# aptx4869lm/4DCapture-FPV

Measured on AMD Instinct MI355X. Metric: frames/sec global-opt (fixed iters), 1024f clip/500k-pt scene; Chamfer GB/s, higher is better.
Workload: dtype f32; 1 GPU; BASELINE config 3: 1024-frame clip, 500000-pt scene, 500 contact verts, 500 Adam iterations (phase split 0.8), full loss; frames sharded over 1 GPU(s); frames=1024, scene_points=500000, contact_verts=500, iters=500, body_verts=10475, lbs_weights_per_vertex=4

## Files before the change

4dcapture-fpv_amd/capi.py:

```python
from __future__ import annotations

import ctypes
import os
from ctypes import POINTER, c_char_p, c_double, c_float, c_int32, c_int64, c_void_p

import numpy as np

_HERE = os.path.dirname(os.path.abspath(__file__))
LIB_PATH = os.environ.get("FDCAP_LIB") or os.path.join(_HERE, "libfdcap_hip.so")

NUM_LOSSES = 8
XDIM = 78
PDIM = 75


class FdcapError(RuntimeError):
    pass


class ModelDesc(ctypes.Structure):
    _fields_ = [("num_verts", c_int32), ("v_template", POINTER(c_float)), ("shapedirs", POINTER(c_float)),
                ("num_shape", c_int32), ("posedirs", POINTER(c_float)), ("J_regressor", POINTER(c_float)),
                ("parents", POINTER(c_int32)), ("lbs_weights", POINTER(c_float)),
                ("hands_componentsl", POINTER(c_float)), ("hands_componentsr", POINTER(c_float)),
# ... 74 lines not shown
    "fdcap_opt_backward_dct": (c_int32, [c_void_p, c_float, c_float, c_float, c_int32, c_void_p]),
    "fdcap_opt_set_dct_coef": (c_int32, [c_void_p, c_void_p, c_void_p]),
    "fdcap_opt_get_dct": (c_int32, [c_void_p, c_void_p, c_void_p]),
    "fdcap_opt_get_dct_state": (c_int32, [c_void_p, c_void_p, c_void_p, c_void_p]),
    "fdcap_opt_set_dct_state": (c_int32, [c_void_p, c_void_p, c_void_p, c_void_p]),
    "fdcap_opt_dct_windows": (c_int32, [c_void_p, POINTER(c_int32), POINTER(c_int32)]),
    "fdcap_frame_smoother": (c_int32, [c_void_p, c_void_p, c_int32, c_int32, c_float, c_float, c_float, c_float,
                                        c_void_p, c_int32, c_int32, c_void_p, c_void_p]),
    "fdcap_opt_set_keypoints": (c_int32, [c_void_p, c_void_p, c_void_p]),
    "fdcap_opt_backward_fit2d": (c_int32, [c_void_p, POINTER(Fit2dStage), c_int32, c_void_p]),
    "fdcap_opt_reset_adam": (c_int32, [c_void_p, c_void_p]),
    "fdcap_lbfgs_create": (c_int32, [c_int32, POINTER(LbfgsConfig), POINTER(c_void_p)]),
    "fdcap_lbfgs_destroy": (None, [c_void_p]),
    "fdcap_lbfgs_reset": (c_int32, [c_void_p, c_void_p]),
    "fdcap_lbfgs_advance": (c_int32, [c_void_p, c_void_p, c_int32, c_void_p, c_void_p, c_int32, c_void_p, c_void_p]),
    "fdcap_lbfgs_get_stats": (c_int32, [c_void_p, c_void_p, c_void_p, c_void_p, c_void_p]),
    "fdcap_lbfgs_finalize": (c_int32, [c_void_p, c_void_p, c_int32, c_void_p, c_void_p]),
    "fdcap_opt_fit2d_lbfgs": (c_int32, [c_void_p, POINTER(Fit2dStage), POINTER(LbfgsConfig), c_int32, POINTER(c_int32), c_void_p]),
    "fdcap_opt_fit2d_lbfgs_stats": (c_int32, [c_void_p, c_void_p, c_void_p, c_void_p, c_void_p]),
    "fdcap_opt_step_rows_and_pack": (c_int32, [c_void_p, c_int32, c_int32, c_void_p, c_void_p]),
    "fdcap_opt_unpack_and_step_scale": (c_int32, [c_void_p, c_int32, c_int32, c_void_p, c_int32, c_int32, c_void_p]),
    "fdcap_opt_forward_ahead": (c_int32, [c_void_p, c_int32, c_int32, c_int32, c_void_p]),
    "fdcap_exchange_len": (c_int32, []),
    "fdcap_opt_get_results": (c_int32, [c_void_p, c_void_p, c_void_p, c_void_p, c_void_p]),
    "fdcap_opt_destroy": (None, [c_void_p]),
    "fdcap_opt_forward_world": (c_int32, [c_void_p, c_void_p, c_void_p, c_void_p]),
    "fdcap_opt_get_contact": (c_int32, [c_void_p, c_void_p, c_void_p, c_void_p]),
    "fdcap_opt_get_grads": (c_int32, [c_void_p, c_void_p, c_void_p, c_void_p]),
    "fdcap_panel_gemm": (c_int32, [c_void_p, c_int32, c_int32, c_int32, c_void_p, c_int64, c_int64, c_int32, c_void_p, c_int32,
                                   c_void_p]),
    "fdcap_time_blend_gemm": (c_int32, [c_void_p, c_int32, c_int32, POINTER(c_float), c_void_p]),
    "fdcap_opt_nn_timing": (c_int32, [c_void_p, c_int32]),
    "fdcap_opt_nn_timing_read": (c_int32, [c_void_p, POINTER(c_float), POINTER(c_int32)]),
    "fdcap_opt_launch_timing": (c_int32, [c_void_p, c_int32]),
    "fdcap_opt_launch_timing_read": (c_int32, [c_void_p, c_void_p, c_void_p]),
    "fdcap_opt_time_chamfer": (c_int32, [c_void_p, c_int32, c_int32, POINTER(c_float), c_void_p]),
}

_lib = None


def load_library(path: str | None = None) -> ctypes.CDLL:
    global _lib
    if _lib is not None and path is None:
        return _lib
    p = path or LIB_PATH
    if not os.path.exists(p):
        raise FdcapError(f"{p} is missing: build it with `python -c 'import __graft_entry__ as g; g.build()'` "
                         "(hipcc --offload-arch=gfx950).  There is no CPU fallback.")
    lib = ctypes.CDLL(p)
    for name, (res, args) in SYMBOLS.items():
        fn = getattr(lib, name)
        fn.restype = res
        fn.argtypes = args
    info = lib.fdcap_build_info().decode()
    if "packed_fp32=off" not in info and os.environ.get("FDCAP_ALLOW_PK_F32") != "1":
        raise FdcapError(f"{p} was built with packed fp32 instructions ({info}): results are not reliable next to another kernel's "
                         "MFMAs on the same CU (NOTES.md section 6).  Rebuild with __graft_entry__.build(), or set "
                         "FDCAP_ALLOW_PK_F32=1 for an instrumentation variant.")
    if path is None:
        _lib = lib
    return lib


def count_packed_fp32(path: str | None = None) -> int:
    import re
# ... 107 lines not shown
```

4dcapture-fpv_amd/csrc/fdc_api_opt.h:

```cpp
#pragma once

extern "C" {

void fdcap_opt_destroy(fdcap_ctx* c) {
    if (!c || !c->opt) return;
    OptState* o = c->opt;
    DevBuf<float>* fb[] = {&o->X0, &o->mask, &o->mX, &o->vX, &o->mCAM, &o->vCAM, &o->mS, &o->vS,
                           &o->H1, &o->H2, &o->O, &o->dO, &o->Opart, &o->dZpart, &o->Rm, &o->PF, &o->Jrest, &o->G, &o->A, &o->M,
                           &o->Jw, &o->Voff, &o->Vw, &o->dist, &o->pd, &o->dVoff, &o->dA, &o->dtransl_v, &o->dMv,
                           &o->dsv, &o->dPF, &o->dJw, &o->dX, &o->dCAM, &o->dscale_row, &o->loss_rows, &o->VoffF, &o->VwF, &o->dVF};
    for (auto* b : fb) b->release();
    o->dctD.release(); o->dctCoef.release(); o->dctM.release(); o->dctV.release(); o->adam_tab.release();
    o->idx.release(); o->pi.release(); o->seedpt.release(); o->kp2d.release(); o->floss.release();
    if (o->lbfgs) { fdcap_lbfgs_destroy(o->lbfgs); o->lbfgs = nullptr; }
    o->nnc_ids.release(); o->nnc_hdr.release(); o->nnc_anchor.release();
    for (hipEvent_t e : o->nn_ev) (void)hipEventDestroy(e);
    o->nn_ev.clear();
    for (hipEvent_t e : o->lt.ev) (void)hipEventDestroy(e);
    o->lt.ev.clear(); o->lt.what.clear(); o->lt.on = false; o->lt.used = 0;
    delete o;
    c->opt = nullptr;
}

int fdcap_opt_create(fdcap_ctx* c, const fdcap_opt_config* cfg, float* rows_x, float* rows_cam, float* scale_d,
// ... 30 lines not shown
    AL(o->X0, (size_t)R * XDIM) AL(o->mask, R)
    AL(o->mX, (size_t)R * XDIM) AL(o->vX, (size_t)R * XDIM) AL(o->mCAM, (size_t)R * 16) AL(o->vCAM, (size_t)R * 16)
    AL(o->mS, 1) AL(o->vS, 1)
    AL(o->H1, (size_t)R * 512) AL(o->H2, (size_t)R * 512) AL(o->O, (size_t)R * O_LD) AL(o->dO, (size_t)R * ODIM)
    AL(o->Opart, (size_t)4 * R * ODIM) AL(o->dZpart, (size_t)4 * R * VP_Z)
    AL(o->Rm, (size_t)R * RM_LD) AL(o->PF, (size_t)R * NPFX) AL(o->Jrest, (size_t)R * JR_LD) AL(o->G, (size_t)R * NJ * 12)
    AL(o->A, (size_t)R * NJ * 12) AL(o->M, (size_t)R * 12) AL(o->Jw, (size_t)R * NJW * 3)
    AL(o->dA, (size_t)R * NJ * 12) AL(o->dtransl_v, (size_t)R * 3) AL(o->dMv, (size_t)R * 12)
    AL(o->dsv, R) AL(o->dPF, (size_t)2 * R * NPFX)
    AL(o->dJw, (size_t)R * NJW * 3) AL(o->dX, (size_t)R * XDIM)
    AL(o->dCAM, (size_t)R * 16) AL(o->dscale_row, R) AL(o->loss_rows, (size_t)R * LROW)
    if (o->contact_on) {
        AL(o->Voff, nq * 3) AL(o->Vw, nq * 3) AL(o->dist, nq) AL(o->idx, nq) AL(o->dVoff, nq * 3) AL(o->seedpt, nq)
        AL(o->pd, (size_t)std::max(o->nsplit, o->nsplit_bf) * nq) AL(o->pi, (size_t)std::max(o->nsplit, o->nsplit_bf) * nq)
    }
#undef AL
    tr.mark("buffers");
    if (!err && o->contact_on) {
        hipError_t e_ = hipMemset(o->idx.p, 0xFF, nq * sizeof(int));
        if (e_ != hipSuccess) err = (int)e_;
    }
    if (!err && o->contact_on) {
        if (const char* e = getenv("FDCAP_SKIN_VEC")) o->skin_vec = e[0] != '0';
        if (const char* e = getenv("FDCAP_FUSE_SKIN")) o->fuse_skin = e[0] != '0';
        if (const char* e = getenv("FDCAP_NN_CACHE_SLACK")) o->nnc_slack = (float)atof(e);
        int every = 32;
        if (const char* e = getenv("FDCAP_NN_ORDER")) every = atoi(e);
        o->nn_order = NNOrder{};
        if (o->nnc_slack > 0.f) {
            const size_t ng = ((size_t)nq_all + 31) / 32, ng4 = ng * 4;
            hipError_t e_ = o->nnc_ids.ensure(ng4 * NN_CACHE_CAP);
            if (e_ == hipSuccess) e_ = o->nnc_hdr.ensure(ng4 + 3 * ng);
            if (e_ == hipSuccess) e_ = o->nnc_anchor.ensure((size_t)4 * nq_all);
            if (e_ == hipSuccess) e_ = hipMemset(o->nnc_hdr.p, 0xFF, ng4 * sizeof(int));
            if (e_ == hipSuccess) e_ = hipMemset(o->nnc_hdr.p + ng4, 0, 3 * ng * sizeof(int));
            if (e_ == hipSuccess) e_ = hipMemset(o->nnc_anchor.p, 0, (size_t)4 * nq_all * sizeof(float4));
            if (e_ != hipSuccess) err = (int)e_;
            if (every > 0) { o->nn_order.on = true; o->nn_order.every = every; }
        }
    }
    if (!err) {
        float s = cfg->scale_init;
        hipError_t e_ = hipMemcpy(o->scale.p, &s, sizeof(float), hipMemcpyHostToDevice);
        if (e_ != hipSuccess) err = (int)e_;
    }
    tr.mark("search state");
    if (err) { fdcap_opt_destroy(c); return err; }
    return FDCAP_OK;
}

int fdcap_opt_set_inputs(fdcap_ctx* c, const float* data78, const float* init78, const float* mask, const float* cam,
                         void* stream) {
    if (!c || !c->opt || !data78 || !init78 || !mask || !cam) return FDCAP_E_ARG;
    { int es_ = opt_sync(c, (hipStream_t)stream); if (es_) return es_; }
    OptState* o = c->opt;
    hipStream_t st = (hipStream_t)stream;
    const size_t n = o->cfg.n_local;
    o->log_pending = false; o->log_dst = nullptr;
    HIP_TRY(hipMemcpyAsync(o->X0.p + 2 * XDIM, data78, n * XDIM * sizeof(float), hipMemcpyDeviceToDevice, st));
    HIP_TRY(hipMemcpyAsync(o->X.p + 2 * XDIM, init78, n * XDIM * sizeof(float), hipMemcpyDeviceToDevice, st));
    HIP_TRY(hipMemcpyAsync(o->mask.p + 2, mask, n * sizeof(float), hipMemcpyDeviceToDevice, st));
    HIP_TRY(hipMemcpyAsync(o->CAM.p + 2 * 16, cam, n * 16 * sizeof(float), hipMemcpyDeviceToDevice, st));
    return FDCAP_OK;
}

static int opt_contact_forward(fdcap_ctx* c, hipStream_t st, bool blend_done = false) {
    OptState* o = c->opt;
    const int nl = o->cfg.n_local, nc = c->nc;
    const size_t off = (size_t)2 * nc * 3;
    const SkinModel smf = c->contact.model();
    const bool fused = !blend_done && o->fuse_skin && gemm_split3_enabled() && c->contact.pn_fwdS.f && smf.vpack && smf.K <= 4 && nl >= clip_forms_min_rows() &&
// ... 190 lines not shown
    if (!c || !c->opt) return FDCAP_E_STATE;
    const fdcap_opt_config& cf = c->opt->cfg;
    const bool phase2 = ii >= P;
    LossWeights lw;
    lw.rec = 1.f;
    lw.smooth = phase2 ? cf.phase2_smooth : cf.phase1_smooth;
    lw.contact = phase2 ? 0.f : cf.phase1_contact;
    lw.world = phase2 ? cf.phase2_world : 0.f;
    lw.dct = 0.f;
    lw.world_on = phase2;
    return opt_backward_impl(c, lw, log_terms, (hipStream_t)stream);
}

int fdcap_opt_backward_and_step(fdcap_ctx* c, int32_t ii, int32_t P, int32_t log_terms, void* stream) {
    if (!c || !c->opt) return FDCAP_E_STATE;
    OptState* o = c->opt;
    const fdcap_opt_config& cf = o->cfg;
    const bool fuse = cf.frame0 == 0 && cf.n_local == cf.n_total && o->dctW == 0;
    if (!fuse) {
        const int e = fdcap_opt_backward(c, ii, P, log_terms, stream);
        return e ? e : fdcap_opt_step(c, ii, P, stream);
    }
    const bool phase2 = ii >= P;
    LossWeights lw;
    lw.rec = 1.f;
    lw.smooth = phase2 ? cf.phase2_smooth : cf.phase1_smooth;
    lw.contact = phase2 ? 0.f : cf.phase1_contact;
    lw.world = phase2 ? cf.phase2_world : 0.f;
    lw.dct = 0.f;
    lw.world_on = phase2;
    return opt_backward_impl(c, lw, log_terms, (hipStream_t)stream, ii, P);
}

}
```

4dcapture-fpv_amd/csrc/fdc_chamfer.h:

```cpp
#pragma once
#include <hip/hip_runtime.h>
#include <stdlib.h>

#include <atomic>

#include "fdc_math.h"

namespace fdc {

constexpr int NN_TILE = 1024;
#ifndef FDC_MF_CH
#define FDC_MF_CH 512
#endif
constexpr int MF_CH = FDC_MF_CH;

struct NNTarget {
    const float4* pts;
    int n;
    const float4* bounds;
    const float4* sbounds;
    const float4* qbounds;
    const int* inv_perm;
    const uint4* frags;
    const float4* centers;
// ... 348 lines not shown
#ifndef FDC_ST4_PF
#define FDC_ST4_PF 2
#endif
#ifndef FDC_AS_MULT
#define FDC_AS_MULT 4.f
#endif
#ifndef FDC_AS_MAX
#define FDC_AS_MAX 3.f
#endif
#ifndef FDC_AS_NEAR
#define FDC_AS_NEAR 0.8f
#endif
#ifndef FDC_ST4_OCC
#define FDC_ST4_OCC 8
#endif
#ifndef FDC_ST4_OCC2
#define FDC_ST4_OCC2 3
#endif
constexpr int ST4_PF = FDC_ST4_PF;
constexpr int ST4_SUPER = 16;
constexpr int ST4_QCAP = 8;

#ifndef FDC_NN_CACHE_CAP
#define FDC_NN_CACHE_CAP 128
#endif
constexpr int NN_CACHE_CAP = FDC_NN_CACHE_CAP;
static_assert(NN_CACHE_CAP == 64 || NN_CACHE_CAP == 128, "one or two ids per lane");
struct NNCache {
    unsigned short* ids;
    int* hdr;
    float4* anchor;
    float slack;
    int order_mode = 0;
};

template <int NQ, int WPG, int WPB = 4>
__global__ __launch_bounds__(64 * WPB, NQ == 1 ? FDC_ST4_OCC : FDC_ST4_OCC2) void nn_stream4_kernel(const float* __restrict__ q, int nq, NNTarget T,
                                                         const int* __restrict__ seed, float4* __restrict__ seedpt,
                                                         float* __restrict__ dist, int* __restrict__ idx, NNCache cache) {
    __shared__ unsigned short slist[WPB][ST4_MAXLIST];
    __shared__ unsigned short clist[WPB][ST4_MAXCELL];
    __shared__ float4 sbox[WPB][64][2];
    __shared__ float s_d[WPB][32 * NQ];
    __shared__ int s_i[WPB][32 * NQ];
    __shared__ float4 s_p[WPB][32 * NQ];
    static_assert(WPG == 1 || WPG == 2 || WPG == 4, "waves per query group");
    static_assert(WPB % WPG == 0 && WPB <= 4, "a group's waves share a workgroup");
    constexpr int GPW = WPB / WPG;
    constexpr int CPS = ST4_SUPER / WPG;
    const int tid = threadIdx.x, wave = tid >> 6, lane = tid & 63, half = lane >> 5, col = lane & 31;
    const int sub = wave % WPG, gslot = wave / WPG;
    const int ngroups = (nq + 32 * NQ - 1) / (32 * NQ);
    const int nwg = (ngroups + GPW - 1) / GPW;
#ifdef FDC_NN_TIMELINE
    const unsigned long long tl_t0 = wall_clock64();
    unsigned long long tl_p[4] = {0, 0, 0, 0};
#define TL_STAMP(k) tl_p[k] = wall_clock64()
#else
#define TL_STAMP(k)
#endif
    const int wg = (cache.order_mode >= 2 && (int)blockIdx.x < nwg) ? cache.hdr[(3 + cache.order_mode) * ((nq + 31) / 32) + (int)blockIdx.x] : (int)blockIdx.x;
    const int group = wg * GPW + gslot;
    const bool idle = wg >= nwg || group >= ngroups;
    const int wq0 = idle ? nq : group * (32 * NQ);
    const int nchunk = (T.n + MF_CH - 1) / MF_CH;
    const int myn = idle ? 0 : (nchunk - sub + WPG - 1) / WPG;
#ifdef FDC_NN_STATS
    unsigned st_cnt[8] = {0, 0, 0, 0, 0, 0, 0, 0};
#endif
    const bool caching = cache.hdr != nullptr && !idle;
    const int cidx = group * WPG + sub;
    float lqx[NQ], lqy[NQ], lqz[NQ];
    int lsj[NQ];
    float4 lsp[NQ];
#pragma unroll
    for (int n = 0; n < NQ; ++n) {
        const size_t qc = (size_t)min(wq0 + n * 32 + col, nq - 1);
        lqx[n] = q[3 * qc]; lqy[n] = q[3 * qc + 1]; lqz[n] = q[3 * qc + 2];
        lsj[n] = seed[qc];
        lsp[n] = seedpt[qc];
    }
    int hv_pre = -1;
    unsigned id_pre = 0;
    float4 anc_pre[NQ];
#pragma unroll
    for (int n = 0; n < NQ; ++n) anc_pre[n] = make_float4(0.f, 0.f, 0.f, -1.f);
    if (caching) {
        hv_pre = cache.hdr[cidx];
        id_pre = NN_CACHE_CAP == 64 ? (unsigned)cache.ids[(size_t)cidx * NN_CACHE_CAP + lane]
                                    : ((const unsigned*)cache.ids)[(size_t)cidx * (NN_CACHE_CAP / 2) + lane];
#pragma unroll
        for (int n = 0; n < NQ; ++n) anc_pre[n] = cache.anchor[(size_t)sub * nq + min(wq0 + n * 32 + col, nq - 1)];
    }
#if defined(__HIP_DEVICE_COMPILE__)
#pragma unroll
    for (int n = 0; n < NQ; ++n)
        asm volatile("" : "+v"(lqx[n]), "+v"(lqy[n]), "+v"(lqz[n]), "+v"(lsj[n]), "+v"(lsp[n].x), "+v"(lsp[n].y), "+v"(lsp[n].z), "+v"(lsp[n].w),
                          "+v"(anc_pre[n].x), "+v"(anc_pre[n].y), "+v"(anc_pre[n].z), "+v"(anc_pre[n].w), "+v"(hv_pre), "+v"(id_pre));
#endif
    float qx[NQ], qy[NQ], qz[NQ], own_d[NQ], sb[NQ];
    int own_i[NQ], qidx[NQ];
    float4 own_p[NQ];
    bool all_seeded = true;
#pragma unroll
    for (int n = 0; n < NQ; ++n) {
        qidx[n] = wq0 + n * 32 + col;
        const bool ok = qidx[n] < nq;
        qx[n] = ok ? lqx[n] : 0.f;
        qy[n] = ok ? lqy[n] : 0.f;
        qz[n] = ok ? lqz[n] : 0.f;
// ... 443 lines not shown
    }
    __syncthreads();
#ifdef FDC_NN_STATS
    {
        unsigned mx = st_cnt[2];
        for (int off = 32; off > 0; off >>= 1) mx = max(mx, (unsigned)__shfl_xor((int)mx, off, 64));
        if (lane == 0 && !idle) {
            atomicAdd(&g_nn_hist[32 + (st_cnt[1] > 0 ? 32 - __clz(st_cnt[1]) : 0)], 1ull);
            atomicAdd(&g_nn_hist[64 + (mx > 0 ? 32 - __clz(mx) : 0)], 1ull);
        }
    }
    for (int i = 0; i < 8; ++i) atomicAdd(&g_nn_stats[i], (unsigned long long)st_cnt[i]);
#endif
#ifdef FDC_NN_TIMELINE
    if (tid == 0 && blockIdx.x < 16384) {
        unsigned xcc; asm volatile("s_getreg_b32 %0, hwreg(HW_REG_XCC_ID)" : "=s"(xcc));
        unsigned long long* tl = g_nn_timeline + (size_t)blockIdx.x * 8;
        tl[0] = tl_t0; tl[1] = wall_clock64(); tl[2] = xcc & 15; tl[3] = tl_p[0]; tl[4] = tl_p[1]; tl[5] = tl_p[2]; tl[6] = tl_p[3]; tl[7] = (unsigned long long)tl_nsurv;
    }
#endif
    if (tid < GPW * 32 * NQ) {
        const int g = tid / (32 * NQ), e = tid % (32 * NQ);
        const int qo = (wg * GPW + g) * (32 * NQ) + e;
        if (wg < nwg && qo < nq) {
            int bw = g * WPG;
            float bd = s_d[bw][e];
            int bi = s_i[bw][e];
#pragma unroll
            for (int w = 1; w < WPG; ++w) {
                const float d = s_d[g * WPG + w][e];
                const int i = s_i[g * WPG + w][e];
                if (i >= 0 && (bi < 0 || nn_better(d, i, bd, bi))) { bd = d; bi = i; bw = g * WPG + w; }
            }
            dist[qo] = bd;
            idx[qo] = bi;
            seedpt[qo] = s_p[bw][e];
        }
    }
}

__global__ __launch_bounds__(256) void nn_seed_kernel(const float* __restrict__ q, int nq, NNTarget T, int* __restrict__ seed,
                                                      float4* __restrict__ seedpt) {
    const int qi = blockIdx.x * 256 + threadIdx.x;
    if (qi >= nq) return;
    const int old = seed[qi];
    if (old >= 0 && old < T.n) {
        const int pos = T.inv_perm ? T.inv_perm[old] : old;
        const float4 pt = T.pts[pos];
        seedpt[qi] = make_float4(pt.x, pt.y, pt.z, __int_as_float(pos));
        return;
    }
    const float x = q[3 * (size_t)qi], y = q[3 * (size_t)qi + 1], z = q[3 * (size_t)qi + 2];
    const int nchunk = (T.n + MF_CH - 1) / MF_CH;
    float bb = INFINITY;
    int bc = -1;
    int p0, p1;
    if (T.sbounds) {
        const int nsuper = (nchunk + ST4_SUPER - 1) / ST4_SUPER;
        for (int s = 0; s < nsuper; ++s) {
            const float ds = box_d2(T.sbounds[2 * s], T.sbounds[2 * s + 1], x, y, z);
            if (!(ds < bb)) continue;
            for (int c = s * ST4_SUPER; c < min(nchunk, (s + 1) * ST4_SUPER); ++c) {
                const float d = box_d2(T.bounds[2 * c], T.bounds[2 * c + 1], x, y, z);
                if (d < bb) { bb = d; bc = c; }
            }
        }
    } else {
        for (int c = 0; c < nchunk; ++c) {
            const float d = box_d2(T.bounds[2 * c], T.bounds[2 * c + 1], x, y, z);
// ... 94 lines not shown
__global__ __launch_bounds__(1024) void nn_order_kernel(const int* __restrict__ work, int n, const int* __restrict__ prev,
                                                        int* __restrict__ order) {
    __shared__ int cnt[16][256], base[256];
    const int tid = threadIdx.x, w = tid >> 6;
    for (int e = tid; e < 16 * 256; e += 1024) (&cnt[0][0])[e] = 0;
    __syncthreads();
    for (int i = tid; i < n; i += 1024) atomicAdd(&cnt[w][255 - min(max(work[i], 0), 255)], 1);
    __syncthreads();
    if (tid < 256) {
        int run = 0;
        for (int k = 0; k < 16; ++k) { const int t = cnt[k][tid]; cnt[k][tid] = run; run += t; }
        base[tid] = run;
    }
    __syncthreads();
    if (tid < 64) {
        const int a = base[4 * tid], b = base[4 * tid + 1], c = base[4 * tid + 2], d = base[4 * tid + 3];
        int s = a + b + c + d, incl = s;
        for (int off = 1; off < 64; off <<= 1) { const int t = __shfl_up(incl, off, 64); if (tid >= off) incl += t; }
        const int ex = incl - s;
        base[4 * tid] = ex; base[4 * tid + 1] = ex + a; base[4 * tid + 2] = ex + a + b; base[4 * tid + 3] = ex + a + b + c;
    }
    __syncthreads();
    for (int i = tid; i < n; i += 1024) {
        const int k = 255 - min(max(work[i], 0), 255);
        order[base[k] + atomicAdd(&cnt[w][k], 1)] = prev ? prev[i] : i;
    }
}
struct NNOrder {
    bool on = false;
    int sorted_groups = 0;
    int cur = 0;
    int age = 0;
    int every = 32;
};

static inline hipError_t nn_search(const float* q, int nq, const NNTarget& T, float* dist, int* idx, float* pd, int* pi,
                                   int nsplit, hipStream_t st, const int* seed = nullptr, bool seed_missing = false,
                                   float4* seedpt = nullptr, bool* seedpt_written = nullptr, const NNCache* cache = nullptr,
                                   NNOrder* ord = nullptr) {
    if (seedpt_written) *seedpt_written = false;
    if (nq <= 0) return hipSuccess;
    const bool culled = seed != nullptr && T.bounds != nullptr;
    static std::atomic<int> use_stream{-1};
    if (use_stream < 0) { const char* e = getenv("FDCAP_NN_STREAM"); use_stream = e ? atoi(e) : -2; }
    if (culled && T.frags != nullptr && use_stream && nn_use_mfma(nq, T.n) && seedpt != nullptr && seed == idx &&
        (T.n + MF_CH - 1) / MF_CH <= 16384) {
        if (seed_missing)
            hipLaunchKernelGGL(nn_seed_kernel, dim3((nq + 255) / 256), dim3(256), 0, st, q, nq, T, idx, seedpt);
        if (seedpt_written) *seedpt_written = true;
        {
            int wpg;
            if (use_stream < 0) {
                const int g32 = (nq + 31) / 32;
                wpg = g32 >= 2816 ? 1 : g32 >= 2304 ? 2 : 4;
            } else {
                wpg = (use_stream / 10 == 4) ? 4 : (use_stream / 10 == 2) ? 2 : 1;
            }
            const int groups = (nq + 31) / 32, wpb = wpg == 1 ? 1 : 4;
            const int nwg = (groups * wpg + wpb - 1) / wpb;
            const dim3 grid((nwg + 7) / 8 * 8);
            NNCache nc = cache ? *cache : NNCache{nullptr, nullptr, nullptr, 0.f};
            const bool ordered = ord != nullptr && ord->on && nc.hdr != nullptr && ord->every > 0 && wpg == 1;
            nc.order_mode = !ordered ? 0 : (ord->sorted_groups == groups ? 2 + ord->cur : 1);
            if (wpg == 4) {
                note_form("nn_stream4_kernel(4 waves per group)");
                hipLaunchKernelGGL((nn_stream4_kernel<1, 4>), grid, dim3(256), 0, st, q, nq, T, seed, seedpt, dist, idx, nc);
            } else if (wpg == 2) {
                note_form("nn_stream4_kernel(2 waves per group)");
                hipLaunchKernelGGL((nn_stream4_kernel<1, 2>), grid, dim3(256), 0, st, q, nq, T, seed, seedpt, dist, idx, nc);
            } else {
                note_form("nn_stream4_kernel<1,1,1>");
                hipLaunchKernelGGL((nn_stream4_kernel<1, 1, 1>), grid, dim3(64), 0, st, q, nq, T, seed, seedpt, dist, idx, nc);
            }
            if (ordered && (ord->sorted_groups != groups || ++ord->age >= ord->every)) {
                const bool had = nc.order_mode >= 2;
                const int nxt = had ? 1 - ord->cur : 0;
                hipLaunchKernelGGL(nn_order_kernel, dim3(1), dim3(1024), 0, st, (const int*)(nc.hdr + 4 * groups), groups,
                                   had ? (const int*)(nc.hdr + (5 + ord->cur) * groups) : (const int*)nullptr, nc.hdr + (5 + nxt) * groups);
                ord->cur = nxt;
                ord->sorted_groups = groups;
                ord->age = 0;
            }
        }
        return hipGetLastError();
    }
    note_form(nn_use_mfma(nq, T.n) ? "nn_mfma_kernel" : "nn_direct_kernel");
    if (nn_use_mfma(nq, T.n) && culled)
        hipLaunchKernelGGL((nn_mfma_kernel<2>), dim3(nn_grid_blocks((nq + 255) / 256, nsplit)), dim3(256), 0, st, q, nq, T, nsplit, seed, pd, pi);
    else if (nn_use_mfma(nq, T.n))
        hipLaunchKernelGGL((nn_mfma_kernel<4>), dim3(nn_grid_blocks((nq + 511) / 512, nsplit)), dim3(256), 0, st, q, nq, T, nsplit, seed, pd, pi);
    else
        hipLaunchKernelGGL((nn_direct_kernel<2>), dim3(nn_grid_blocks((nq + 511) / 512, nsplit)), dim3(256), 0, st, q, nq, T, nsplit, pd, pi);
    hipLaunchKernelGGL(nn_combine_kernel, dim3((nq + 255) / 256), dim3(256), 0, st, pd, pi, nsplit, nq, dist, idx);
    return hipGetLastError();
}

}
```

4dcapture-fpv_amd/csrc/fdc_scene.h:

```cpp
#pragma once
#include <hip/hip_runtime.h>

#include <algorithm>
#include <utility>
#include <vector>

#include "fdc_chamfer.h"

namespace fdc {

constexpr int SC_RS_ROUNDS = 16;
constexpr int SC_RS_TILE = 256 * SC_RS_ROUNDS;
constexpr int SC_PT_TILE = 1024;
constexpr int SC_SUPER = 16;

__device__ __forceinline__ unsigned sc_key(float v) {
    unsigned u = __float_as_uint(v);
    if ((u << 1) == 0u) u = 0u;
    return (u & 0x80000000u) ? ~u : (u | 0x80000000u);
}

__global__ __launch_bounds__(256) void sc_keys_kernel(const float* __restrict__ xyz, int n, int axis, unsigned* __restrict__ keys,
                                                      int* __restrict__ vals) {
    const int i = blockIdx.x * 256 + threadIdx.x;
    if (i < n) { keys[i] = sc_key(xyz[3 * (size_t)i + axis]); vals[i] = i; }
}

__global__ __launch_bounds__(256) void sc_rs_hist_kernel(const unsigned* __restrict__ keys, int n, int shift, unsigned* __restrict__ hist, int nb) {
    __shared__ unsigned h[256];
    h[threadIdx.x] = 0;
    __syncthreads();
    const int base = blockIdx.x * SC_RS_TILE;
    for (int r = 0; r < SC_RS_ROUNDS; ++r) {
        const int i = base + r * 256 + threadIdx.x;
        if (i < n) atomicAdd(&h[(keys[i] >> shift) & 255u], 1u);
    }
    __syncthreads();
    hist[(size_t)threadIdx.x * nb + blockIdx.x] = h[threadIdx.x];
}

__global__ __launch_bounds__(1024) void sc_scan_kernel(unsigned* __restrict__ a, int m) {
    __shared__ unsigned part[1024];
    a += (size_t)blockIdx.x * m;
    const int per = (m + 1023) / 1024;
    const int lo = min(m, (int)threadIdx.x * per), hi = min(m, lo + per);
    unsigned s = 0;
    for (int i = lo; i < hi; ++i) s += a[i];
    part[threadIdx.x] = s;
    __syncthreads();
    for (int o = 1; o < 1024; o <<= 1) {
        unsigned t = threadIdx.x >= (unsigned)o ? part[threadIdx.x - o] : 0u;
        __syncthreads();
        part[threadIdx.x] += t;
        __syncthreads();
    }
    unsigned run = part[threadIdx.x] - s;
    for (int i = lo; i < hi; ++i) { unsigned v = a[i]; a[i] = run; run += v; }
}

__global__ __launch_bounds__(256) void sc_rs_scatter_kernel(const unsigned* __restrict__ kin, const int* __restrict__ vin,
                                                            unsigned* __restrict__ kout, int* __restrict__ vout, int n, int shift,
                                                            const unsigned* __restrict__ hist, int nb) {
    __shared__ unsigned base[256];
    __shared__ unsigned wcnt[4][256];
    const int tid = threadIdx.x, wave = tid >> 6, lane = tid & 63;
    base[tid] = hist[(size_t)tid * nb + blockIdx.x];
    const int tile0 = blockIdx.x * SC_RS_TILE;
    for (int r = 0; r < SC_RS_ROUNDS; ++r) {
        const int i = tile0 + r * 256 + tid;
        const bool valid = i < n;
        const unsigned key = valid ? kin[i] : 0u;
        const int val = valid ? vin[i] : 0;
        const unsigned d = (key >> shift) & 255u;
        unsigned long long m = __ballot(valid);
#pragma unroll
        for (int b = 0; b < 8; ++b) {
            const bool bit = (d >> b) & 1u;
            const unsigned long long bal = __ballot(bit);
            m &= bit ? bal : ~bal;
        }
        const int rank = __popcll(m & ((1ull << lane) - 1ull));
        for (int k = 0; k < 4; ++k) wcnt[k][tid] = 0;
        __syncthreads();
        if (valid && rank == 0) wcnt[wave][d] = (unsigned)__popcll(m);
        __syncthreads();
        if (valid) {
            unsigned off = base[d];
            for (int k = 0; k < wave; ++k) off += wcnt[k][d];
            kout[off + rank] = key;
            vout[off + rank] = val;
        }
        __syncthreads();
        base[tid] += wcnt[0][tid] + wcnt[1][tid] + wcnt[2][tid] + wcnt[3][tid];
        __syncthreads();
    }
}

__device__ __forceinline__ int sc_find_node(const int4* __restrict__ nodes, int nn, int p) {
    int lo = 0, hi = nn - 1;
    while (lo < hi) {
        const int mid = (lo + hi + 1) >> 1;
        if (nodes[mid].x <= p) lo = mid; else hi = mid - 1;
    }
    return lo;
}

__global__ __launch_bounds__(256) void sc_axis_kernel(const int4* __restrict__ nodes, int nn, const float* __restrict__ xyz,
                                                      const int* __restrict__ Lx, const int* __restrict__ Ly, const int* __restrict__ Lz,
                                                      unsigned char* __restrict__ axis) {
    const int i = blockIdx.x * 256 + threadIdx.x;
    if (i >= nn) return;
    const int4 nd = nodes[i];
    int ax = 0;
    if (nd.z < nd.y) {
        const int a = nd.x, b = nd.x + nd.y - 1;
        const float ex = xyz[3 * (size_t)Lx[b]] - xyz[3 * (size_t)Lx[a]];
        const float ey = xyz[3 * (size_t)Ly[b] + 1] - xyz[3 * (size_t)Ly[a] + 1];
        const float ez = xyz[3 * (size_t)Lz[b] + 2] - xyz[3 * (size_t)Lz[a] + 2];
        float best = ex;
        if (ey > best) { ax = 1; best = ey; }
        if (ez > best) { ax = 2; }
    }
    axis[i] = (unsigned char)ax;
}

__global__ __launch_bounds__(256) void sc_side_kernel(const int4* __restrict__ nodes, int nn, const unsigned char* __restrict__ axis,
                                                      const int* __restrict__ Lx, const int* __restrict__ Ly, const int* __restrict__ Lz,
                                                      int n, unsigned char* __restrict__ side) {
// ... 306 lines not shown
```

4dcapture-fpv_amd/csrc/fdc_state.h:

```cpp
#pragma once

namespace {

struct SetupTrace {
    bool on;
    const char* who;
    std::chrono::steady_clock::time_point t0, last;
    explicit SetupTrace(const char* w) : who(w) {
        const char* e = getenv("FDCAP_SETUP_TRACE");
        on = e && e[0] == '1';
        if (on) t0 = last = std::chrono::steady_clock::now();
    }
    void mark(const char* what) {
        if (!on) return;
        (void)hipDeviceSynchronize();
        const auto now = std::chrono::steady_clock::now();
        fprintf(stderr, "[fdcap setup] %s: %-28s %8.3f ms (at %8.3f)\n", who, what, std::chrono::duration<double, std::milli>(now - last).count(),
                std::chrono::duration<double, std::milli>(now - t0).count());
        last = now;
    }
};

template <class T>
struct DevBuf {
// ... 67 lines not shown
                     pn_fwd3_f.release(); pn_bwd3_f.release(); pn_fwd3_s.release(); pn_bwd3_s.release(); pn_fwdS_f.release(); pn_fwdS_s.release(); pn_fwdS = PanelB3(); pn_fwd3 = PanelB3(); pn_bwd3 = PanelB3(); }
};

struct OptState {
    fdcap_opt_config cfg;
    int R = 0;
    bool contact_on = false;
    int nsplit = 8;
    int nsplit_bf = 8;
    struct Ext { float* p = nullptr; } X, CAM, scale, dscale;
    struct ExtD { double* p = nullptr; } losses;
    DevBuf<float> X0, mask, mX, vX, mCAM, vCAM, mS, vS;
    struct { bool on = false; int ii = 0, P = 0; } pend;
    DevBuf<float> H1, H2, O, dO;
    DevBuf<float> Opart, dZpart;
    bool dz_pending = false;
    DevBuf<float> Rm, PF, Jrest, G, A, M, Jw;
    DevBuf<float> Voff, Vw, dist, pd, dVoff;
    DevBuf<int> idx, pi;
    DevBuf<float> kp2d;
    DevBuf<float> floss;
    fdcap_lbfgs* lbfgs = nullptr;
    DevBuf<float4> seedpt;
    bool skin_vec = true;
    bool fuse_skin = true;
    DevBuf<float> loss_rows;
    bool log_pending = false;
    unsigned log_mask = 0;
    int log_assign = 0;
    double* log_dst = nullptr;
    DevBuf<unsigned short> nnc_ids;
    DevBuf<int> nnc_hdr;
    DevBuf<float4> nnc_anchor;
    NNOrder nn_order;
    float nnc_slack = 0.03f;
    struct LaunchTimes {
        bool on = false;
        int used = 0, phase = 0;
        std::vector<hipEvent_t> ev;
        std::vector<signed char> what;
    } lt;
    bool nn_timing = false;
    std::vector<hipEvent_t> nn_ev;
    int nn_ev_used = 0;
    NNCache nn_cache(int) { return NNCache{nnc_slack > 0.f ? nnc_ids.p : nullptr, nnc_slack > 0.f ? nnc_hdr.p : nullptr, nnc_anchor.p, nnc_slack}; }
    DevBuf<float> dA, dtransl_v, dMv, dsv, dPF, dJw, dX, dCAM, dscale_row;
    DevBuf<float> VoffF, VwF, dVF;
    int cam_steps = 0;
    DevBuf<float> dctD, dctCoef, dctM, dctV;
    DevBuf<AdamScalars> adam_tab;
    std::vector<AdamScalars> adam_tab_h;
    int dctT = 0, dctC = 0, dctW = 0;
    bool dct_grad = false;
    bool seeded = false;
    bool ahead = false, ahead_blend = false;
    bool nnpt_valid = false;
    bool use_seed = true;
    bool use_cull = true;
};

inline void lt_mark(OptState* o, int what, hipStream_t st) {
    OptState::LaunchTimes& t = o->lt;
    if (!t.on || t.used >= (int)t.ev.size()) return;
    if (hipEventRecord(t.ev[t.used], st) != hipSuccess) return;
    t.what[t.used++] = (signed char)(what < 0 ? -1 : what + 16 * t.phase);
}
// ... 490 lines not shown
```

include/fdcap.h:

```cpp
#ifndef FDCAP_H
#define FDCAP_H

#include <stdint.h>

#ifdef __cplusplus
extern "C" {
#endif

#define FDCAP_OK 0
#define FDCAP_E_ARG (-1)
#define FDCAP_E_STATE (-2)
#define FDCAP_E_NODEVICE (-3)
#define FDCAP_E_COMM (-4)
#define FDCAP_UNIQUE_ID_BYTES 128

#define FDCAP_NUM_JOINTS 55
#define FDCAP_XDIM 78
#define FDCAP_PDIM 75
#define FDCAP_MAX_SCENE_POINTS 67000000
#define FDCAP_NUM_LOSSES 8

typedef struct fdcap_ctx fdcap_ctx;

typedef struct fdcap_model_desc {
// ... 141 lines not shown
int fdcap_opt_fit2d_lbfgs_stats(fdcap_ctx* ctx, int32_t* iterations_d, int32_t* evaluations_d, float* loss_d, void* stream);

int fdcap_opt_step_rows_and_pack(fdcap_ctx* ctx, int32_t ii, int32_t first_phase2_iter, float* send_d, void* stream);
int fdcap_opt_unpack_and_step_scale(fdcap_ctx* ctx, int32_t ii, int32_t first_phase2_iter, const float* gathered_d,
                                    int32_t rank, int32_t world, void* stream);
int32_t fdcap_exchange_len(void);

int fdcap_comm_unique_id(uint8_t* id128);
int fdcap_comm_create(fdcap_ctx* ctx, const uint8_t* id128, int32_t rank, int32_t world);
int fdcap_comm_destroy(fdcap_ctx* ctx);
const char* fdcap_comm_last_error(fdcap_ctx* ctx);
int fdcap_opt_halo_exchange(fdcap_ctx* ctx, void* stream);
int fdcap_opt_exchange(fdcap_ctx* ctx, int32_t ii, int32_t first_phase2_iter, void* stream);
int fdcap_opt_time_exchange(fdcap_ctx* ctx, int32_t iters, float* us_exchange, float* us_allgather, void* stream);
int fdcap_comm_allreduce_f64(fdcap_ctx* ctx, double* buf_d, int32_t n, void* stream);
int fdcap_opt_forward_ahead(fdcap_ctx* ctx, int32_t ii, int32_t first_phase2_iter, int32_t log_terms, void* stream);

int fdcap_opt_get_results(fdcap_ctx* ctx, float* body_rec75_d, float* scale_d, float* cam_ext_d,
                          void* stream);
void fdcap_opt_destroy(fdcap_ctx* ctx);

int fdcap_opt_forward_world(fdcap_ctx* ctx, float* verts_d, float* joints_d, void* stream);
int fdcap_opt_get_contact(fdcap_ctx* ctx, float* dist_d, int32_t* idx_d, void* stream);
int fdcap_opt_get_grads(fdcap_ctx* ctx, float* dx_d, float* dcam_d, void* stream);

int fdcap_time_blend_gemm(fdcap_ctx* ctx, int32_t rows, int32_t iters, float* ms, void* stream);

int fdcap_panel_gemm(const float* A_d, int32_t lda, int32_t M, int32_t K, const float* B_h, int64_t sk, int64_t sn, int32_t N,
                     float* C_d, int32_t ldc, void* stream);

int fdcap_opt_nn_timing(fdcap_ctx* ctx, int32_t max_launches);
int fdcap_opt_nn_timing_read(fdcap_ctx* ctx, float* mean_ms, int32_t* launches);

#define FDCAP_LT_VPOSER_FWD 0
#define FDCAP_LT_POSE_FWD 1
#define FDCAP_LT_CONTACT_FWD 2
#define FDCAP_LT_CHAMFER_NN 3
#define FDCAP_LT_SKIN_BWD 4
#define FDCAP_LT_BLEND_BWD 5
#define FDCAP_LT_POSE_BWD 6
#define FDCAP_LT_VPOSER_BWD 7
#define FDCAP_LT_NUM 8
int fdcap_opt_launch_timing(fdcap_ctx* ctx, int32_t max_events);
int fdcap_opt_launch_timing_read(fdcap_ctx* ctx, float* mean_us , int32_t* counts );

int fdcap_opt_time_chamfer(fdcap_ctx* ctx, int32_t iters, int32_t brute_force, float* ms, void* stream);

#ifdef __cplusplus
}
#endif
#endif
```

Baseline: 17500 frames/s.

## Reorder NN queries by seed scene position via radix sort for locality

Adds a query permutation for the Chamfer nearest-neighbour stream kernel. The queries are radix-sorted by their cached seed point's scene position, so that neighbouring lanes and waves search spatially coherent regions. The sort reuses the scene radix-sort kernels and is redone when the group ordering would otherwise be resorted. The single-block scan kernel also batches its loads into unrolled chunks of 16. A debug entry point can force identity, no permutation or a host-supplied permutation. The permutation adds indirect gathers and scatters plus extra shared memory per wave, and reordering resets the group ordering state.

```diff
diff --git a/4dcapture-fpv_amd/capi.py b/4dcapture-fpv_amd/capi.py
--- a/4dcapture-fpv_amd/capi.py
+++ b/4dcapture-fpv_amd/capi.py
@@ -130,6 +130,7 @@
     "fdcap_time_blend_gemm": (c_int32, [c_void_p, c_int32, c_int32, POINTER(c_float), c_void_p]),
     "fdcap_opt_nn_timing": (c_int32, [c_void_p, c_int32]),
     "fdcap_opt_nn_timing_read": (c_int32, [c_void_p, POINTER(c_float), POINTER(c_int32)]),
+    "fdcap_debug_nn_query_order": (c_int32, [c_void_p, c_int32, c_void_p, c_int32]),
     "fdcap_opt_launch_timing": (c_int32, [c_void_p, c_int32]),
     "fdcap_opt_launch_timing_read": (c_int32, [c_void_p, c_void_p, c_void_p]),
     "fdcap_opt_time_chamfer": (c_int32, [c_void_p, c_int32, c_int32, POINTER(c_float), c_void_p]),
diff --git a/4dcapture-fpv_amd/csrc/fdc_api_opt.h b/4dcapture-fpv_amd/csrc/fdc_api_opt.h
--- a/4dcapture-fpv_amd/csrc/fdc_api_opt.h
+++ b/4dcapture-fpv_amd/csrc/fdc_api_opt.h
@@ -86,11 +86,12 @@
             hipError_t e_ = o->nnc_ids.ensure(ng4 * NN_CACHE_CAP);
             if (e_ == hipSuccess) e_ = o->nnc_hdr.ensure(ng4 + 3 * ng);
             if (e_ == hipSuccess) e_ = o->nnc_anchor.ensure((size_t)4 * nq_all);
+            if (e_ == hipSuccess && every > 0) e_ = o->nnq_buf.ensure(nn_query_order_ints(nq_all));
             if (e_ == hipSuccess) e_ = hipMemset(o->nnc_hdr.p, 0xFF, ng4 * sizeof(int));
             if (e_ == hipSuccess) e_ = hipMemset(o->nnc_hdr.p + ng4, 0, 3 * ng * sizeof(int));
             if (e_ == hipSuccess) e_ = hipMemset(o->nnc_anchor.p, 0, (size_t)4 * nq_all * sizeof(float4));
             if (e_ != hipSuccess) err = (int)e_;
-            if (every > 0) { o->nn_order.on = true; o->nn_order.every = every; }
+            if (every > 0) { o->nn_order.on = true; o->nn_order.every = every; o->nn_order.qbuf = o->nnq_buf.p; }
         }
     }
     if (!err) {
@@ -347,4 +348,29 @@
     return opt_backward_impl(c, lw, log_terms, (hipStream_t)stream, ii, P);
 }
 
-}
+int fdcap_debug_nn_query_order(fdcap_ctx* c, int32_t mode, const int32_t* perm_host, int32_t n) {
+    if (!c || !c->opt) return FDCAP_E_STATE;
+    if (mode < 0 || mode > 2) return FDCAP_E_ARG;
+    OptState* o = c->opt;
+    NNOrder& ord = o->nn_order;
+    if (!o->contact_on || ord.qbuf == nullptr) return FDCAP_E_STATE;
+    const int nq = o->cfg.n_local * c->nc;
+    if (mode == 2) {
+        if (!perm_host || n != nq) return FDCAP_E_ARG;
+        std::vector<char> seen((size_t)nq, 0);
+        for (int i = 0; i < nq; ++i) {
+            if (perm_host[i] < 0 || perm_host[i] >= nq || seen[perm_host[i]]) return FDCAP_E_ARG;
+            seen[perm_host[i]] = 1;
+        }
+    }
+    HIP_TRY(hipDeviceSynchronize());
+    if (mode == 2) HIP_TRY(hipMemcpy(ord.qbuf, perm_host, (size_t)nq * sizeof(int), hipMemcpyHostToDevice));
+    HIP_TRY(hipMemset(o->nnc_hdr.p, 0xFF, (size_t)(nq + 31) / 32 * sizeof(int)));
+    ord.perm_mode = mode;
+    ord.perm_n = mode == 2 ? nq : 0;
+    ord.sorted_groups = 0;
+    ord.age = 0;
+    return FDCAP_OK;
+}
+
+}
diff --git a/4dcapture-fpv_amd/csrc/fdc_chamfer.h b/4dcapture-fpv_amd/csrc/fdc_chamfer.h
--- a/4dcapture-fpv_amd/csrc/fdc_chamfer.h
+++ b/4dcapture-fpv_amd/csrc/fdc_chamfer.h
@@ -404,6 +404,7 @@
     float4* anchor;
     float slack;
     int order_mode = 0;
+    const int* perm = nullptr;
 };
 
 template <int NQ, int WPG, int WPB = 4>
@@ -416,6 +417,7 @@
     __shared__ float s_d[WPB][32 * NQ];
     __shared__ int s_i[WPB][32 * NQ];
     __shared__ float4 s_p[WPB][32 * NQ];
+    __shared__ int s_q[WPB][32 * NQ];
     static_assert(WPG == 1 || WPG == 2 || WPG == 4, "waves per query group");
     static_assert(WPB % WPG == 0 && WPB <= 4, "a group's waves share a workgroup");
     constexpr int GPW = WPB / WPG;
@@ -445,9 +447,14 @@
     float lqx[NQ], lqy[NQ], lqz[NQ];
     int lsj[NQ];
     float4 lsp[NQ];
+    const int* const perm = NQ == 1 && WPB == 1 ? cache.perm : nullptr;
 #pragma unroll
     for (int n = 0; n < NQ; ++n) {
-        const size_t qc = (size_t)min(wq0 + n * 32 + col, nq - 1);
+        size_t qc = (size_t)min(wq0 + n * 32 + col, nq - 1);
+        if (perm) {
+            qc = (size_t)perm[qc];
+            if (half == 0) s_q[wave][n * 32 + col] = (int)qc;
+        }
         lqx[n] = q[3 * qc]; lqy[n] = q[3 * qc + 1]; lqz[n] = q[3 * qc + 2];
         lsj[n] = seed[qc];
         lsp[n] = seedpt[qc];
@@ -957,9 +964,10 @@
                 const int i = s_i[g * WPG + w][e];
                 if (i >= 0 && (bi < 0 || nn_better(d, i, bd, bi))) { bd = d; bi = i; bw = g * WPG + w; }
             }
-            dist[qo] = bd;
-            idx[qo] = bi;
-            seedpt[qo] = s_p[bw][e];
+            const int qd = perm ? s_q[g][e] : qo;
+            dist[qd] = bd;
+            idx[qd] = bi;
+            seedpt[qd] = s_p[bw][e];
         }
     }
 }
@@ -1120,7 +1128,12 @@
     int cur = 0;
     int age = 0;
     int every = 32;
+    int* qbuf = nullptr;
+    int perm_n = 0;
+    int perm_mode = 0;
 };
+static inline size_t nn_query_order_ints(int nq);
+static inline hipError_t nn_query_order(const float4* seedpt, int nq, int* qbuf, int* hdr, int groups, hipStream_t st);
 
 static inline hipError_t nn_search(const float* q, int nq, const NNTarget& T, float* dist, int* idx, float* pd, int* pi,
                                    int nsplit, hipStream_t st, const int* seed = nullptr, bool seed_missing = false,
@@ -1150,6 +1163,8 @@
             NNCache nc = cache ? *cache : NNCache{nullptr, nullptr, nullptr, 0.f};
             const bool ordered = ord != nullptr && ord->on && nc.hdr != nullptr && ord->every > 0 && wpg == 1;
             nc.order_mode = !ordered ? 0 : (ord->sorted_groups == groups ? 2 + ord->cur : 1);
+            const bool qorder = ordered && ord->qbuf != nullptr && ord->perm_mode != 1;
+            nc.perm = qorder && ord->perm_n == nq ? ord->qbuf : nullptr;
             if (wpg == 4) {
                 note_form("nn_stream4_kernel(4 waves per group)");
                 hipLaunchKernelGGL((nn_stream4_kernel<1, 4>), grid, dim3(256), 0, st, q, nq, T, seed, seedpt, dist, idx, nc);
@@ -1160,7 +1175,14 @@
                 note_form("nn_stream4_kernel<1,1,1>");
                 hipLaunchKernelGGL((nn_stream4_kernel<1, 1, 1>), grid, dim3(64), 0, st, q, nq, T, seed, seedpt, dist, idx, nc);
             }
-            if (ordered && (ord->sorted_groups != groups || ++ord->age >= ord->every)) {
+            const bool resort = ordered && (ord->sorted_groups != groups || ++ord->age >= ord->every);
+            if (qorder && ord->perm_mode == 0 && (ord->perm_n != nq || seed_missing || (resort && ord->sorted_groups == groups))) {
+                const hipError_t e = nn_query_order(seedpt, nq, ord->qbuf, nc.hdr, groups, st);
+                if (e != hipSuccess) return e;
+                ord->perm_n = nq;
+                ord->sorted_groups = 0;
+                ord->age = 0;
+            } else if (resort) {
                 const bool had = nc.order_mode >= 2;
                 const int nxt = had ? 1 - ord->cur : 0;
                 hipLaunchKernelGGL(nn_order_kernel, dim3(1), dim3(1024), 0, st, (const int*)(nc.hdr + 4 * groups), groups,
diff --git a/4dcapture-fpv_amd/csrc/fdc_scene.h b/4dcapture-fpv_amd/csrc/fdc_scene.h
--- a/4dcapture-fpv_amd/csrc/fdc_scene.h
+++ b/4dcapture-fpv_amd/csrc/fdc_scene.h
@@ -11,6 +11,7 @@
 
 constexpr int SC_RS_ROUNDS = 16;
 constexpr int SC_RS_TILE = 256 * SC_RS_ROUNDS;
+constexpr int SC_SCAN_BATCH = 16;
 constexpr int SC_PT_TILE = 1024;
 constexpr int SC_SUPER = 16;
 
@@ -45,7 +46,13 @@
     const int per = (m + 1023) / 1024;
     const int lo = min(m, (int)threadIdx.x * per), hi = min(m, lo + per);
     unsigned s = 0;
-    for (int i = lo; i < hi; ++i) s += a[i];
+    for (int i0 = lo; i0 < hi; i0 += SC_SCAN_BATCH) {
+        unsigned v[SC_SCAN_BATCH];
+#pragma unroll
+        for (int k = 0; k < SC_SCAN_BATCH; ++k) v[k] = i0 + k < hi ? a[i0 + k] : 0u;
+#pragma unroll
+        for (int k = 0; k < SC_SCAN_BATCH; ++k) s += v[k];
+    }
     part[threadIdx.x] = s;
     __syncthreads();
     for (int o = 1; o < 1024; o <<= 1) {
@@ -55,7 +62,14 @@
         __syncthreads();
     }
     unsigned run = part[threadIdx.x] - s;
-    for (int i = lo; i < hi; ++i) { unsigned v = a[i]; a[i] = run; run += v; }
+    for (int i0 = lo; i0 < hi; i0 += SC_SCAN_BATCH) {
+        unsigned v[SC_SCAN_BATCH];
+#pragma unroll
+        for (int k = 0; k < SC_SCAN_BATCH; ++k) v[k] = i0 + k < hi ? a[i0 + k] : 0u;
+#pragma unroll
+        for (int k = 0; k < SC_SCAN_BATCH; ++k)
+            if (i0 + k < hi) { a[i0 + k] = run; run += v[k]; }
+    }
 }
 
 __global__ __launch_bounds__(256) void sc_rs_scatter_kernel(const unsigned* __restrict__ kin, const int* __restrict__ vin,
@@ -94,6 +108,36 @@
         base[tid] += wcnt[0][tid] + wcnt[1][tid] + wcnt[2][tid] + wcnt[3][tid];
         __syncthreads();
     }
+}
+
+static inline size_t nn_query_order_ints(int nq) { return 4 * (size_t)nq + 256 * (size_t)((nq + SC_RS_TILE - 1) / SC_RS_TILE); }
+
+__global__ __launch_bounds__(256) void nn_order_keys_kernel(const float4* __restrict__ seedpt, int nq, unsigned* __restrict__ key,
+                                                            int* __restrict__ val, int* __restrict__ hdr, int groups) {
+    const int i = blockIdx.x * 256 + threadIdx.x;
+    if (i < nq) {
+        const int pos = __float_as_int(seedpt[i].w);
+        key[i] = pos >= 0 ? min((unsigned)pos >> 7, 0xFFFFu) : 0xFFFFu;
+        val[i] = i;
+    }
+    if (i < groups) hdr[i] = -1;
+}
+
+static inline hipError_t nn_query_order(const float4* seedpt, int nq, int* qbuf, int* hdr, int groups, hipStream_t st) {
+    const int nb = (nq + SC_RS_TILE - 1) / SC_RS_TILE;
+    int* const perm = qbuf;
+    int* const val = qbuf + nq;
+    unsigned* const key = (unsigned*)(qbuf + 2 * (size_t)nq);
+    unsigned* const hist = key + 2 * (size_t)nq;
+    hipLaunchKernelGGL(nn_order_keys_kernel, dim3((std::max(nq, groups) + 255) / 256), dim3(256), 0, st, seedpt, nq, key, perm, hdr, groups);
+    for (int pass = 0; pass < 2; ++pass) {
+        unsigned* const kin = key + (size_t)pass * nq;
+        unsigned* const kout = key + (size_t)(1 - pass) * nq;
+        hipLaunchKernelGGL(sc_rs_hist_kernel, dim3(nb), dim3(256), 0, st, kin, nq, 8 * pass, hist, nb);
+        hipLaunchKernelGGL(sc_scan_kernel, dim3(1), dim3(1024), 0, st, hist, 256 * nb);
+        hipLaunchKernelGGL(sc_rs_scatter_kernel, dim3(nb), dim3(256), 0, st, kin, pass ? val : perm, kout, pass ? perm : val, nq, 8 * pass, hist, nb);
+    }
+    return hipGetLastError();
 }
 
 __device__ __forceinline__ int sc_find_node(const int4* __restrict__ nodes, int nn, int p) {
diff --git a/4dcapture-fpv_amd/csrc/fdc_state.h b/4dcapture-fpv_amd/csrc/fdc_state.h
--- a/4dcapture-fpv_amd/csrc/fdc_state.h
+++ b/4dcapture-fpv_amd/csrc/fdc_state.h
@@ -123,6 +123,7 @@
     DevBuf<unsigned short> nnc_ids;
     DevBuf<int> nnc_hdr;
     DevBuf<float4> nnc_anchor;
+    DevBuf<int> nnq_buf;
     NNOrder nn_order;
     float nnc_slack = 0.03f;
     struct LaunchTimes {
diff --git a/include/fdcap.h b/include/fdcap.h
--- a/include/fdcap.h
+++ b/include/fdcap.h
@@ -197,6 +197,8 @@
 int fdcap_opt_nn_timing(fdcap_ctx* ctx, int32_t max_launches);
 int fdcap_opt_nn_timing_read(fdcap_ctx* ctx, float* mean_ms, int32_t* launches);
 
+int fdcap_debug_nn_query_order(fdcap_ctx* ctx, int32_t mode, const int32_t* perm_h, int32_t n);
+
 #define FDCAP_LT_VPOSER_FWD 0
 #define FDCAP_LT_POSE_FWD 1
 #define FDCAP_LT_CONTACT_FWD 2
```

New measurement: 17940 frames/s, median of 6. 2.5% higher.
